# JuanTarrio/rebvo

Measured on AMD Instinct MI355X. Metric: frames/sec (DoG+extract+track+depth) 752x480 EuRoC, higher is better.
Workload: dtype f32 scale-space / f64 tracker+EKF

## Files before the change

rebvo_amd/csrc/stage_b.hip:

```cpp

#include <math.h>
#include <string.h>

#include <vector>

#include <type_traits>

#include "ctx.h"
#include "wave_reduce.h"

namespace edgehip {

struct RetuneArgs {
    SeqA *seqa;
    const int32_t *histo;
    float *retuned_out;
    int knum, nbins;
};
template <int NT>
__global__ __launch_bounds__(NT) void k_quantile(const KlSoA *kls, const int32_t *__restrict__ kns, SeqDev *seqs,
                                                 double smin, double smax, double pct, int nbins, const double *__restrict__ t_in, double fps,
                                                 RetuneArgs rt) {
    __shared__ int s_h[256];
    const int seq = blockIdx.x, tid = threadIdx.x;
// ... 502 lines not shown
    R[0] = 1.0 - B * (wy2 + wz2);
    R[4] = 1.0 - B * (wx2 + wz2);
    R[8] = 1.0 - B * (wx2 + wy2);
    double a = A * w[2], b = B * (w[0] * w[1]);
    R[1] = b - a; R[3] = b + a;
    a = A * w[1]; b = B * (w[0] * w[2]);
    R[2] = b + a; R[6] = b - a;
    a = A * w[0]; b = B * (w[1] * w[2]);
    R[5] = b - a; R[7] = b + a;
}
__device__ __noinline__ void so3_exp(const double w[3], double R[9]) {
    const double wv[3] = {w[0], w[1], w[2]};
    double Rr[9];
    so3_exp_inl(wv, Rr);
    for (int i = 0; i < 9; i++) R[i] = Rr[i];
}

__device__ __noinline__ void tvr_setup(SeqDev *sq, const double *X) {
    double R0[9], Rz[9];
    so3_exp(X + 3, R0);
    const double wz[3] = {0.0, 0.0, X[5]};
    so3_exp(wz, Rz);
    for (int i = 0; i < 9; i++) sq->Rt[i] = R0[i];
    sq->RM[0] = Rz[0]; sq->RM[1] = Rz[1]; sq->RM[2] = Rz[3]; sq->RM[3] = Rz[4];
    for (int i = 0; i < 3; i++) sq->Vt[i] = X[i];
}


__device__ __forceinline__ void tvr_setup2(SeqDev *sq, const double *X, const int lane, const bool zero = false, const int l0 = 0) {
    if (lane >= l0 && lane < l0 + 2) {
        const bool first = lane == l0;
        const double wv[3] = {first ? X[3] : 0.0, first ? X[4] : 0.0, X[5]};
        double R[9];
        so3_exp_inl(wv, R);
        double *Rt = zero ? sq->zRt : sq->Rt, *Vt = zero ? sq->zVt : sq->Vt, *RM = zero ? sq->zRM : sq->RM;
        if (first) {
            for (int i = 0; i < 9; i++) Rt[i] = R[i];
            for (int i = 0; i < 3; i++) Vt[i] = X[i];
        } else {
            RM[0] = R[0]; RM[1] = R[1]; RM[2] = R[3]; RM[3] = R[4];
        }
    }
}


struct TvrArgs {
    const KlSoA *kl_old;
    const KlSoA *kl_new;
    const int32_t *kn_old;
    const uint16_t *field16;
    const double *P0;
    double *resid;
    double *resid_carry;
    double *block_last;
    double *partials;
    double *block_last_z;
    double *partials_z;
    SeqDev *seq;
    const uint32_t *framecount;
    int w, h, cap, nblk, nseq;
    size_t f16stride;
    int f16tx;
    double zfm, max_r, match_thresh, k_huber, inv_k_huber;
    double inv_zfm;
    float ppx, ppy;
    uint32_t match_num_thresh;
    int write_mid;
    int use_grec;
    unsigned long long *fwd_key;
    const edgehip_kf_request *kf;
    double kf_match_mod, kf_match_cang, kf_rho_tol;
};

__device__ __forceinline__ double rsqrt_f64(double x) {
    double y = __builtin_amdgcn_rsq(x);
    const double hx = 0.5 * x;
    y = y * (1.5 - hx * y * y);
    y = y * (1.5 - hx * y * y);
    return x > 1e300 ? 0.0 : y;
}

__device__ __forceinline__ bool is_carry(double v) { return __double_as_longlong(v) == (long long)resid_carry_bits(); }

#ifndef EDGEHIP_TVR_MFMA
#define EDGEHIP_TVR_MFMA 0
#endif
#ifndef EDGEHIP_TVR_REF_ORDER
#define EDGEHIP_TVR_REF_ORDER 1
#endif
#ifndef EDGEHIP_TVR_ABL
#define EDGEHIP_TVR_ABL 0
#endif
template <bool REWEIGHT, bool PROCJF, bool GREC, bool KF = false>
__device__ __forceinline__ void tvr_body(const TvrArgs &a, const int seq, const int blk, const int tid) {
    constexpr int ABL = KF ? 0 : EDGEHIP_TVR_ABL;
    const int lane = tid & 63, wave = tid >> 6;
    SeqDev *sq = a.seq + seq;
    const int kn = a.kn_old[seq];
    if (blk * kTvrBlock >= kn) return;
    const KlSoA &ko = a.kl_old[seq];
    const int res_in = sq->res_cur, res_out = sq->lm_phase == 0 ? sq->res_t : sq->res_new;
    const double *rin = a.resid + ((size_t)res_in * a.nseq + seq) * a.cap;
    double *rout = a.resid + ((size_t)res_out * a.nseq + seq) * a.cap;
    const double carry_in_prev = a.resid_carry[((size_t)res_in * a.nseq + seq) * a.nblk + blk];
    const double marker = __longlong_as_double((long long)resid_carry_bits());

    constexpr int NW = kTvrThreads / 64;
    constexpr bool GRAM_MFMA = PROCJF && kTvrPasses == 1 && EDGEHIP_TVR_MFMA && !(ABL & 1);
    __shared__ double s_rows[GRAM_MFMA ? NW : 1][GRAM_MFMA ? 64 : 1][8];
    __shared__ double s_wlast[kTvrPasses][NW];
    __shared__ int s_whas[kTvrPasses][NW];
    double sums[kNumSums];
#pragma unroll
    for (int i = 0; i < kNumSums; i++) sums[i] = 0;

#pragma unroll 1
    for (int pass = 0; pass < kTvrPasses; pass++) {
        const int base = blk * kTvrBlock + pass * kTvrThreads;
        if (base >= kn) break;
        const int ikl = base + tid;
        double J[6] = {0, 0, 0, 0, 0, 0};
        double fm, dfx, dfy;
        double ptx, pty, ptz, pix, piy, rho_p, s_rho;
#if EDGEHIP_TVR_REF_ORDER
        double wgt_ref;
#else
        double inv_w2 = 1;
#endif
        int mid_f = -1;
        int status = 0;
        double fi = 0;
        double rho_own;
        if (ikl < kn) {
            s_rho = ldg(ko.s_rho, ikl);
            const int32_t mnum = ldg(ko.m_num, ikl);
            const float2 pm0 = ldg(ko.p_m, ikl);
            const double rho0 = ldg(ko.rho, ikl);
            rho_own = rho0;
            const float2 klm = ldg(ko.m_m, ikl);
            const float knm = ldg(ko.n_m, ikl);
            double rprev = 0;
            if (REWEIGHT && !(ABL & 16)) rprev = rin[ikl];
            const uint32_t fc = KF ? 0xFFFFFFFFu : a.framecount[seq];
            const uint32_t mthr = a.match_num_thresh < fc ? a.match_num_thresh : fc;
            const bool skip = s_rho > sq->s_rho_min_eval || (uint32_t)mnum < mthr;
            if (!skip) {
                const double sz = inv_mid(rho0);
                const double pz_zf0 = a.inv_zfm * sz;
                const double sx = pz_zf0 * (double)pm0.x, sy = pz_zf0 * (double)pm0.y;
                const double *R = sq->Rt, *V = sq->Vt;
                ptx = R[0] * sx; ptx += R[1] * sy; ptx += R[2] * sz; ptx = V[0] + ptx;
                pty = R[3] * sx; pty += R[4] * sy; pty += R[5] * sz; pty = V[1] + pty;
                ptz = R[6] * sx; ptz += R[7] * sy; ptz += R[8] * sz; ptz = V[2] + ptz;
                rho_p = inv_mid(ptz);
                const double pz_zf = a.zfm * rho_p;
                pix = pz_zf * ptx;
                piy = pz_zf * pty;
                const double px = pix + (double)a.ppx, py = piy + (double)a.ppy;
                const int x = cvt_trunc_sat_i32(px + 0.5), y = cvt_trunc_sat_i32(py + 0.5);
                dfx = 0; dfy = 0;
#if EDGEHIP_TVR_REF_ORDER
                wgt_ref = 1;
#endif
                if (REWEIGHT) {
                    if (is_carry(rprev)) rprev = carry_in_prev;
#if EDGEHIP_TVR_REF_ORDER
                    if (fabs(rprev) > a.k_huber) wgt_ref = div_mid(a.k_huber, fabs(rprev));
#else
                    if (fabs(rprev) > a.k_huber && !(ABL & 2)) { const double rk = fabs(rprev) * a.inv_k_huber; inv_w2 = rk * rk; }
#endif
                }
                fm = a.max_r;
                if (x < 1 || y < 1 || x >= a.w - 1 || y >= a.h - 1) {
                    status = 1;
                } else {
                    status = 3;
                    const float rmx = KF ? klm.x : (float)(sq->RM[0] * (double)klm.x + sq->RM[1] * (double)klm.y);
                    const float rmy = KF ? klm.y : (float)(sq->RM[2] * (double)klm.x + sq->RM[3] * (double)klm.y);
                    const uint32_t f = (ABL & 8) ? (uint32_t)(ikl + 1) : a.field16[(size_t)seq * a.f16stride + field16_index(x, y, a.f16tx)];
                    if (KF) {
                        if (f != 0u) {
                            const int ikf = (int)f - 1;
                            const KlSoA &kf = a.kl_new[seq];
                            const MatchRec fr = kf.rec[ikf];
                            const double f_rho = kf.rho[ikf], f_srho = kf.s_rho[ikf];
                            const double cang = (double)((klm.x * fr.m_mx + klm.y * fr.m_my) / knm);
                            const double rho_t = rho_p / a.kf[seq].Kr;
                            const bool reject = cang < a.kf_match_cang || (double)fabsf(knm / fr.n_m - 1) > a.kf_match_mod ||
                                                fabs(rho_t - f_rho) > a.kf_rho_tol * (f_srho + s_rho * rho_t / rho0);
                            if (!reject) {
                                const double dx = px - (double)fr.c_px, dy = py - (double)fr.c_py;
                                fi = dx * (double)fr.u_mx + dy * (double)fr.u_my;
// ... 39 lines not shown

        {
            const unsigned long long vmask = __ballot(status == 2);
            const unsigned long long below = vmask & ((1ull << lane) - 1ull);
            const int src = below ? 63 - __clzll(below) : 0;
            const double inh = __shfl(fi, src, 64);
            const int top = vmask ? 63 - __clzll(vmask) : 0;
            const double wl = __shfl(fi, top, 64);
            if (lane == 0) {
                s_whas[pass][wave] = vmask != 0;
                s_wlast[pass][wave] = wl;
            }
            __syncthreads();
            if (status == 3) {
                double v = marker;
                bool have = false;
                if (below) { v = inh; have = true; }
                for (int pp = pass; pp >= 0 && !have; pp--)
                    for (int pw = (pp == pass ? wave - 1 : NW - 1); pw >= 0 && !have; pw--)
                        if (s_whas[pp][pw]) { v = s_wlast[pp][pw]; have = true; }
                rout[ikl] = v;
            } else if (status == 2) {
                rout[ikl] = fi;
            } else if (status == 1) {
                rout[ikl] = a.max_r;
            } else if (ikl < kn) {
                rout[ikl] = 0.0;
            }
        }
        if (a.write_mid && ikl < kn) {
            stg(ko.m_id_f, ikl, mid_f);
            if (!KF && a.fwd_key && mid_f >= 0) atomicMax(&a.fwd_key[(size_t)seq * a.cap + mid_f], ord_bits(rho_own));
        }

        double fs = 0;
        if (status != 0) {
#if EDGEHIP_TVR_REF_ORDER
            if (REWEIGHT) { fm *= wgt_ref; dfx *= wgt_ref; dfy *= wgt_ref; }
#endif
            if (PROCJF) {
                double t0 = a.zfm * rho_p;
                J[0] = t0 * dfx;
                J[1] = t0 * dfy;
                t0 = rho_p * pix;
                J[2] = t0 * dfx;
                t0 = rho_p * piy;
                J[2] += t0 * dfy;
                J[3] = J[1] * ptz; J[3] += J[2] * pty;
                J[4] = J[0] * ptz; J[4] += J[2] * ptx;
                t0 = J[0] * pty;
                J[5] = -1 * t0; J[5] += J[1] * ptx;
            }
            const double qvel = (a.zfm * dfx * sq->Vt[0] + a.zfm * dfy * sq->Vt[1] + (pix * dfx + piy * dfy) * sq->Vt[2]);
#if EDGEHIP_TVR_REF_ORDER
            const double q_rho = REWEIGHT ? sqrt_ge1(s_rho * qvel * s_rho * qvel + 1) : s_rho;
            const double r_q = rcp_for_div_rn(q_rho);
            if (PROCJF) {
#pragma unroll
                for (int j = 0; j < 6; j++) J[j] = div_rn(J[j], q_rho, r_q);
            }
            fs = div_rn(fm, q_rho, r_q);
#else
            double inv_q;
            if (REWEIGHT) {
                const double sq = s_rho * qvel;
                inv_q = (ABL & 2) ? sq + inv_w2 : rsqrt_f64(sq * sq + inv_w2);
            } else {
                inv_q = 1.0 / s_rho;
            }
            if (PROCJF) {
#pragma unroll
                for (int j = 0; j < 6; j++) J[j] *= inv_q;
            }
            fs = fm * inv_q;
#endif
        } else if (!REWEIGHT && !KF && ikl < kn && s_rho == 0) {
            const double qnan = __longlong_as_double(0x7ff8000000000000ll);
            if (PROCJF) {
#pragma unroll
                for (int j = 0; j < 6; j++) J[j] = qnan;
            }
            fs = qnan;
        }
        if (GRAM_MFMA) {
            double2 *row = reinterpret_cast<double2 *>(&s_rows[wave][lane][0]);
            row[0] = make_double2(J[0], J[1]);
            row[1] = make_double2(J[2], J[3]);
            row[2] = make_double2(J[4], J[5]);
            row[3] = make_double2(fs, 0.0);
        } else {
            int ns = 0;
            if (PROCJF) {
#pragma unroll
                for (int i = 0; i < 6; i++)
#pragma unroll
                    for (int j = i; j < 6; j++) { const double pr = J[i] * J[j]; sums[ns] = kTvrPasses == 1 ? pr : sums[ns] + pr; ns++; }
#pragma unroll
                for (int i = 0; i < 6; i++) { const double pr = J[i] * fs; sums[ns] = kTvrPasses == 1 ? pr : sums[ns] + pr; ns++; }
            }
            { const double pr = fs * fs; const int at = PROCJF ? ns : kNumSums - 1; sums[at] = kTvrPasses == 1 ? pr : sums[at] + pr; }
        }
    }

    if (tid == 0) {
        double bl = marker;
        for (int pp = kTvrPasses - 1; pp >= 0 && is_carry(bl); pp--) {
            if (blk * kTvrBlock + pp * kTvrThreads >= kn) continue;
            for (int pw = NW - 1; pw >= 0; pw--)
                if (s_whas[pp][pw]) { bl = s_wlast[pp][pw]; break; }
        }
        a.block_last[(size_t)seq * a.nblk + blk] = bl;
    }

    __shared__ double s_red[NW][32];
    if (GRAM_MFMA) {
        typedef double v4d __attribute__((ext_vector_type(4)));
        __builtin_amdgcn_fence(__ATOMIC_RELEASE, "wavefront");
        __builtin_amdgcn_wave_barrier();
        const int m = (lane & 15) < 7 ? (lane & 15) : 7, kk = lane >> 4;
        const double *src = &s_rows[wave][kk][m];
        v4d acc = {0.0, 0.0, 0.0, 0.0};
#pragma unroll
        for (int st = 0; st < 16; st++) {
            const double v = src[st * 4 * 8];
            acc = __builtin_amdgcn_mfma_f64_16x16x4f64(v, v, acc, 0, 0, 0);
        }
        const int j = lane & 15;
#pragma unroll
        for (int r = 0; r < 2; r++) {
            const int i = (lane >> 4) + 4 * r;
            if (j < 7 && i <= j) {
                const int idx = j < 6 ? i * 6 - (i * (i - 1)) / 2 + (j - i) : (i < 6 ? 21 + i : 27);
                s_red[wave][idx] = acc[r];
            }
        }
    } else if (PROCJF && (ABL & 1)) {
        if (lane < kNumSums) s_red[wave][lane] = sums[lane % 4];
    } else if (PROCJF) {
        const int idx = wave_reduce28(sums, lane);
        if ((lane & 1) == 0) s_red[wave][idx] = sums[0];
    } else {
        double v = sums[kNumSums - 1];
#pragma unroll
        for (int o = 32; o > 0; o >>= 1) v += __shfl_xor(v, o, 64);
        if (lane == 0) s_red[wave][kNumSums - 1] = v;
    }
    __syncthreads();
    if (PROCJF ? tid < kNumSums : tid == kNumSums - 1) {
        double v = s_red[0][tid];
#pragma unroll
        for (int wv = 1; wv < NW; wv++) v += s_red[wv][tid];
        a.partials[((size_t)seq * a.nblk + blk) * kNumSums + tid] = v;
    }
}

template <bool REWEIGHT, bool PROCJF, bool GREC>
__global__ __launch_bounds__(kTvrThreads) void k_try_velrot(TvrArgs a) {
    tvr_body<REWEIGHT, PROCJF, GREC>(a, blockIdx.z, blockIdx.x, threadIdx.x);
}
__global__ __launch_bounds__(kTvrThreads) void k_try_velrot_kf(TvrArgs a) {
    tvr_body<true, true, false, true>(a, blockIdx.z, blockIdx.x, threadIdx.x);
}

template <bool REWEIGHT, bool PROCJF, bool GREC>
__device__ __forceinline__ void tvr_body_f32(const TvrArgs &a, const int seq, const int blk, const int tid) {
    static_assert(kTvrPasses == 1, "one KeyLine per thread");
    const int lane = tid & 63, wave = tid >> 6;
    SeqDev *sq = a.seq + seq;
    const int kn = a.kn_old[seq];
    if (blk * kTvrBlock >= kn) return;
    const KlSoA &ko = a.kl_old[seq];
    const int res_in = sq->res_cur, res_out = sq->lm_phase == 0 ? sq->res_t : sq->res_new;
    const double *rin = a.resid + ((size_t)res_in * a.nseq + seq) * a.cap;
    double *rout = a.resid + ((size_t)res_out * a.nseq + seq) * a.cap;
    const double carry_in_prev = a.resid_carry[((size_t)res_in * a.nseq + seq) * a.nblk + blk];
    const double marker = __longlong_as_double((long long)resid_carry_bits());
    constexpr int NW = kTvrThreads / 64;
    __shared__ float s_wlast[NW];
    __shared__ int s_whas[NW];
    float sums[kNumSums];
#pragma unroll
    for (int i = 0; i < kNumSums; i++) sums[i] = 0.f;

    const int ikl = blk * kTvrBlock + tid;
    float J[6] = {0, 0, 0, 0, 0, 0};
    float fm, dfx, dfy;
    float ptx, pty, ptz, pix, piy, rho_p;
    double s_rho;
    float wgt;
    int mid_f = -1, status = 0;
    float fi = 0;
    double rho_own;
    const float zf = (float)a.zfm, max_r = (float)a.max_r, k_huber = (float)a.k_huber, simil_t = (float)a.match_thresh;
    float Vt0, Vt1, Vt2;
    if (ikl < kn) {
        s_rho = ldg(ko.s_rho, ikl);
        const int32_t mnum = ldg(ko.m_num, ikl);
        const float2 pm0 = ldg(ko.p_m, ikl);
        const double rho0 = ldg(ko.rho, ikl);
        rho_own = rho0;
        const float2 klm = ldg(ko.m_m, ikl);
        const float knm = ldg(ko.n_m, ikl);
        double rprev_d = 0;
        if (REWEIGHT) rprev_d = rin[ikl];
        const uint32_t fc = a.framecount[seq];
        const uint32_t mthr = a.match_num_thresh < fc ? a.match_num_thresh : fc;
        const bool skip = s_rho > sq->s_rho_min_eval || (uint32_t)mnum < mthr;
        Vt0 = (float)sq->Vt[0]; Vt1 = (float)sq->Vt[1]; Vt2 = (float)sq->Vt[2];
        if (!skip) {
            const float sz = 1.f / (float)rho0;
            const float pz_zf0 = (1.f / zf) * sz;
            const float sx = pz_zf0 * pm0.x, sy = pz_zf0 * pm0.y;
            const double *Rd = sq->Rt;
            const float R0 = (float)Rd[0], R1 = (float)Rd[1], R2 = (float)Rd[2], R3 = (float)Rd[3], R4 = (float)Rd[4], R5 = (float)Rd[5],
                        R6 = (float)Rd[6], R7 = (float)Rd[7], R8 = (float)Rd[8];
            ptx = R0 * sx; ptx += R1 * sy; ptx += R2 * sz; ptx = Vt0 + ptx;
            pty = R3 * sx; pty += R4 * sy; pty += R5 * sz; pty = Vt1 + pty;
            ptz = R6 * sx; ptz += R7 * sy; ptz += R8 * sz; ptz = Vt2 + ptz;
            rho_p = 1.f / ptz;
            const float pz_zf = zf * rho_p;
            pix = pz_zf * ptx;
            piy = pz_zf * pty;
            const float px = pix + a.ppx, py = piy + a.ppy;
            const int x = cvt_trunc_sat_i32((double)px + 0.5), y = cvt_trunc_sat_i32((double)py + 0.5);
            dfx = 0; dfy = 0; wgt = 1;
            if (REWEIGHT) {
                if (is_carry(rprev_d)) rprev_d = carry_in_prev;
                const float rprev = (float)rprev_d;
                if (fabsf(rprev) > k_huber) wgt = k_huber / fabsf(rprev);
            }
            fm = max_r;
            if (x < 1 || y < 1 || x >= a.w - 1 || y >= a.h - 1) {
                status = 1;
            } else {
                status = 3;
                const float rmx = (float)sq->RM[0] * klm.x + (float)sq->RM[1] * klm.y;
                const float rmy = (float)sq->RM[2] * klm.x + (float)sq->RM[3] * klm.y;
                const uint32_t f = a.field16[(size_t)seq * a.f16stride + field16_index(x, y, a.f16tx)];
                {
                    const int ikf = f != 0u ? (int)f - 1 : 0;
                    float f_cpx, f_cpy, f_mx, f_my, f_ux, f_uy;
                    if (GREC) {
                        const float4 g = ldg(a.kl_new[seq].grec, ikf);
// ... 39 lines not shown
            bool have = false;
            if (below) { v = (double)inh; have = true; }
            for (int pw = wave - 1; pw >= 0 && !have; pw--)
                if (s_whas[pw]) { v = (double)s_wlast[pw]; have = true; }
            rout[ikl] = v;
        } else if (status == 2) {
            rout[ikl] = (double)fi;
        } else if (status == 1) {
            rout[ikl] = (double)max_r;
        } else if (ikl < kn) {
            rout[ikl] = 0.0;
        }
    }
    if (a.write_mid && ikl < kn) {
        stg(ko.m_id_f, ikl, mid_f);
        if (a.fwd_key && mid_f >= 0) atomicMax(&a.fwd_key[(size_t)seq * a.cap + mid_f], ord_bits(rho_own));
    }
    float fs = 0.f;
    if (status != 0) {
        if (REWEIGHT) { fm *= wgt; dfx *= wgt; dfy *= wgt; }
        if (PROCJF) {
            float t0 = zf * rho_p;
            J[0] = t0 * dfx;
            J[1] = t0 * dfy;
            t0 = rho_p * pix;
            J[2] = t0 * dfx;
            t0 = rho_p * piy;
            J[2] += t0 * dfy;
            J[3] = J[1] * ptz; J[3] += J[2] * pty;
            J[4] = J[0] * ptz; J[4] += J[2] * ptx;
            t0 = J[0] * pty;
            J[5] = -1.f * t0; J[5] += J[1] * ptx;
        }
        const double qvel = (double)(zf * dfx * Vt0 + zf * dfy * Vt1 + (pix * dfx + piy * dfy) * Vt2);
        const double q_rho = REWEIGHT ? sqrt_ge1(s_rho * qvel * s_rho * qvel + 1) : s_rho;
        const double r_q = rcp_for_div_rn(q_rho);
        if (PROCJF) {
#pragma unroll
            for (int j = 0; j < 6; j++) J[j] = (float)div_rn((double)J[j], q_rho, r_q);
        }
        fs = (float)div_rn((double)fm, q_rho, r_q);
    }
    {
        int ns = 0;
        if (PROCJF) {
#pragma unroll
            for (int i = 0; i < 6; i++)
#pragma unroll
                for (int j = i; j < 6; j++) sums[ns++] = J[i] * J[j];
#pragma unroll
            for (int i = 0; i < 6; i++) sums[ns++] = J[i] * fs;
        }
        sums[PROCJF ? ns : kNumSums - 1] = fs * fs;
    }
    if (tid == 0) {
        double bl = marker;
        for (int pw = NW - 1; pw >= 0; pw--)
            if (s_whas[pw]) { bl = (double)s_wlast[pw]; break; }
        a.block_last[(size_t)seq * a.nblk + blk] = bl;
    }
    __shared__ float s_red[NW][32];
    if (PROCJF) {
        const int idx = wave_reduce28_f32(sums, lane);
        if ((lane & 1) == 0) s_red[wave][idx] = sums[0];
    } else {
        float v = sums[kNumSums - 1];
#pragma unroll
        for (int o = 32; o > 0; o >>= 1) v += __shfl_xor(v, o, 64);
        if (lane == 0) s_red[wave][kNumSums - 1] = v;
    }
    __syncthreads();
    if (PROCJF ? tid < kNumSums : tid == kNumSums - 1) {
        float v = s_red[0][tid];
#pragma unroll
        for (int wv = 1; wv < NW; wv++) v += s_red[wv][tid];
        a.partials[((size_t)seq * a.nblk + blk) * kNumSums + tid] = (double)v;
    }
}
template <bool REWEIGHT, bool PROCJF, bool GREC>
__global__ __launch_bounds__(kTvrThreads) void k_try_velrot_f32(TvrArgs a) {
    tvr_body_f32<REWEIGHT, PROCJF, GREC>(a, blockIdx.z, blockIdx.x, threadIdx.x);
}

#ifndef EDGEHIP_TVR2_PARK
#define EDGEHIP_TVR2_PARK 1
#endif
template <bool PROCJF, bool GREC>
__device__ __forceinline__ void tvr2_body(const TvrArgs &a, const int seq, const int blk, const int tid) {
    const int lane = tid & 63, wave = tid >> 6;
    SeqDev *sq = a.seq + seq;
    const int kn = a.kn_old[seq];
    if (blk * kTvrBlock >= kn) return;
    static_assert(kTvrPasses == 1, "one KeyLine per thread");
    const KlSoA &ko = a.kl_old[seq];
    double *rout0 = a.resid + ((size_t)sq->res_t * a.nseq + seq) * a.cap;
    double *rout1 = a.resid + ((size_t)sq->res_new * a.nseq + seq) * a.cap;
    const double marker = __longlong_as_double((long long)resid_carry_bits());
    constexpr int NW = kTvrThreads / 64;
    __shared__ double s_wlast[2][NW];
    __shared__ int s_whas[2][NW];

    const int ikl = blk * kTvrBlock + tid;
    double fm[2], dfx[2], dfy[2], fi[2] = {0, 0};
    double ptx[2], pty[2], ptz[2], pix[2], piy[2], rho_p[2];
    int status[2] = {0, 0};
    double s_rho = 1;
    if (ikl < kn) {
        s_rho = ldg(ko.s_rho, ikl);
        const int32_t mnum = ldg(ko.m_num, ikl);
        const float2 pm0 = ldg(ko.p_m, ikl);
        const double rho0 = ldg(ko.rho, ikl);
        const float2 klm = ldg(ko.m_m, ikl);
        const float knm = ldg(ko.n_m, ikl);
        const uint32_t fc = a.framecount[seq];
        const uint32_t mthr = a.match_num_thresh < fc ? a.match_num_thresh : fc;
        const bool skip = s_rho > sq->s_rho_min_eval || (uint32_t)mnum < mthr;
        if (!skip) {
            const double sz = inv_mid(rho0);
            const double pz_zf0 = a.inv_zfm * sz;
            const double sx = pz_zf0 * (double)pm0.x, sy = pz_zf0 * (double)pm0.y;
            double px[2], py[2];
            bool inimg[2];
            size_t fidx[2];
            float rmx[2], rmy[2];
#pragma unroll
            for (int c = 0; c < 2; c++) {
                const double *R = c ? sq->Rt : sq->zRt, *V = c ? sq->Vt : sq->zVt, *RM = c ? sq->RM : sq->zRM;
                ptx[c] = R[0] * sx; ptx[c] += R[1] * sy; ptx[c] += R[2] * sz; ptx[c] = V[0] + ptx[c];
                pty[c] = R[3] * sx; pty[c] += R[4] * sy; pty[c] += R[5] * sz; pty[c] = V[1] + pty[c];
                ptz[c] = R[6] * sx; ptz[c] += R[7] * sy; ptz[c] += R[8] * sz; ptz[c] = V[2] + ptz[c];
                rho_p[c] = inv_mid(ptz[c]);
                const double pz_zf = a.zfm * rho_p[c];
                pix[c] = pz_zf * ptx[c];
                piy[c] = pz_zf * pty[c];
                px[c] = pix[c] + (double)a.ppx; py[c] = piy[c] + (double)a.ppy;
                const int x = x86_cvttsd2si(px[c] + 0.5), y = x86_cvttsd2si(py[c] + 0.5);
                inimg[c] = !(x < 1 || y < 1 || x >= a.w - 1 || y >= a.h - 1);
                fidx[c] = inimg[c] ? field16_index(x, y, a.f16tx) : (size_t)0;
                rmx[c] = (float)(RM[0] * (double)klm.x + RM[1] * (double)klm.y);
                rmy[c] = (float)(RM[2] * (double)klm.x + RM[3] * (double)klm.y);
                fm[c] = a.max_r;
                dfx[c] = 0; dfy[c] = 0;
                status[c] = inimg[c] ? 3 : 1;
            }
            const uint16_t *fld = a.field16 + (size_t)seq * a.f16stride;
            const uint32_t f0 = fld[fidx[0]], f1 = fld[fidx[1]];
            const bool hit0 = inimg[0] && f0 != 0u, hit1 = inimg[1] && f1 != 0u;
            const int ikf0 = hit0 ? (int)f0 - 1 : 0, ikf1 = hit1 ? (int)f1 - 1 : 0;
            float f_cpx[2], f_cpy[2], f_mx[2], f_my[2], f_ux[2] = {0, 0}, f_uy[2] = {0, 0};
            if (GREC) {
                const float4 g0 = ldg(a.kl_new[seq].grec, ikf0), g1 = ldg(a.kl_new[seq].grec, ikf1);
                f_cpx[0] = g0.x; f_cpy[0] = g0.y; f_mx[0] = g0.z; f_my[0] = g0.w;
                f_cpx[1] = g1.x; f_cpy[1] = g1.y; f_mx[1] = g1.z; f_my[1] = g1.w;
            } else {
                const MatchRec r0 = a.kl_new[seq].rec[ikf0], r1 = a.kl_new[seq].rec[ikf1];
                f_cpx[0] = r0.c_px; f_cpy[0] = r0.c_py; f_mx[0] = r0.m_mx; f_my[0] = r0.m_my; f_ux[0] = r0.u_mx; f_uy[0] = r0.u_my;
                f_cpx[1] = r1.c_px; f_cpy[1] = r1.c_py; f_mx[1] = r1.m_mx; f_my[1] = r1.m_my; f_ux[1] = r1.u_mx; f_uy[1] = r1.u_my;
            }
            const double p_n2 = (double)(knm * knm);
#pragma unroll
            for (int c = 0; c < 2; c++) {
                {
                    const double p_esc = (double)(rmx[c] * f_mx[c] + rmy[c] * f_my[c]);
                    if ((c ? hit1 : hit0) & !(fabs(p_esc - p_n2) > a.match_thresh * p_n2)) {
                        if (GREC) {
                            const float n2m = f_mx[c] * f_mx[c] + f_my[c] * f_my[c];
                            const float nm = sqrtf_mid(n2m);
                            div2_mid_f32(f_mx[c], f_my[c], nm, f_ux[c], f_uy[c]);
                        }
                        const double dx = px[c] - (double)f_cpx[c], dy = py[c] - (double)f_cpy[c];
                        fi[c] = dx * (double)f_ux[c] + dy * (double)f_uy[c];
                        dfx[c] = (double)f_ux[c];
                        dfy[c] = (double)f_uy[c];
                        fm[c] = fi[c];
                        status[c] = 2;
                    }
                }
            }
        }
    }

    unsigned long long below[2];
    double inh[2];
#pragma unroll
    for (int c = 0; c < 2; c++) {
        const unsigned long long vmask = __ballot(status[c] == 2);
        below[c] = vmask & ((1ull << lane) - 1ull);
        const int src = below[c] ? 63 - __clzll(below[c]) : 0;
        inh[c] = __shfl(fi[c], src, 64);
        const int top = vmask ? 63 - __clzll(vmask) : 0;
        const double wl = __shfl(fi[c], top, 64);
        if (lane == 0) {
            s_whas[c][wave] = vmask != 0;
            s_wlast[c][wave] = wl;
        }
    }
    __syncthreads();
#pragma unroll
    for (int c = 0; c < 2; c++) {
        double *rout = c ? rout1 : rout0;
        if (status[c] == 3) {
            double v = marker;
            bool have = false;
            if (below[c]) { v = inh[c]; have = true; }
            for (int pw = wave - 1; pw >= 0 && !have; pw--)
                if (s_whas[c][pw]) { v = s_wlast[c][pw]; have = true; }
            rout[ikl] = v;
        } else if (status[c] == 2) {
            rout[ikl] = fi[c];
        } else if (status[c] == 1) {
            rout[ikl] = a.max_r;
        } else if (ikl < kn) {
            rout[ikl] = 0.0;
        }
    }
    if (tid == 0) {
#pragma unroll
        for (int c = 0; c < 2; c++) {
            double bl = marker;
            for (int pw = NW - 1; pw >= 0; pw--)
                if (s_whas[c][pw]) { bl = s_wlast[c][pw]; break; }
            (c ? a.block_last : a.block_last_z)[(size_t)seq * a.nblk + blk] = bl;
        }
    }

    __shared__ double s_red[2][NW][32];
#if EDGEHIP_TVR2_PARK
    __shared__ double s_park[PROCJF ? 7 : 1][kTvrThreads];
#endif
    const double inv_q = rcp_for_div_rn(s_rho);
    double Jc[2][6], fmc[2];
#pragma unroll
    for (int c = 0; c < 2; c++) {
        double *J = Jc[c];
#pragma unroll
        for (int j = 0; j < 6; j++) J[j] = 0;
        fmc[c] = 0;
        if (status[c] != 0) {
            fmc[c] = fm[c];
            if (PROCJF) {
                double t0 = a.zfm * rho_p[c];
                J[0] = t0 * dfx[c];
                J[1] = t0 * dfy[c];
                t0 = rho_p[c] * pix[c];
                J[2] = t0 * dfx[c];
                t0 = rho_p[c] * piy[c];
                J[2] += t0 * dfy[c];
                J[3] = J[1] * ptz[c]; J[3] += J[2] * pty[c];
                J[4] = J[0] * ptz[c]; J[4] += J[2] * ptx[c];
                t0 = J[0] * pty[c];
                J[5] = -1 * t0; J[5] += J[1] * ptx[c];
#if EDGEHIP_TVR_REF_ORDER
#pragma unroll
                for (int j = 0; j < 6; j++) J[j] = div_rn(J[j], s_rho, inv_q);
#else
#pragma unroll
                for (int j = 0; j < 6; j++) J[j] *= inv_q;
#endif
            }
#if EDGEHIP_TVR_REF_ORDER
            fmc[c] = div_rn(fmc[c], s_rho, inv_q);
#else
            fmc[c] *= inv_q;
#endif
        } else if (ikl < kn && s_rho == 0) {
            const double qnan = __longlong_as_double(0x7ff8000000000000ll);
            if (PROCJF) {
#pragma unroll
                for (int j = 0; j < 6; j++) J[j] = qnan;
            }
            fmc[c] = qnan;
        }
    }
#if EDGEHIP_TVR2_PARK
    if (PROCJF) {
#pragma unroll
        for (int j = 0; j < 6; j++) s_park[j][tid] = Jc[1][j];
        s_park[6][tid] = fmc[1];
    }
#endif
#pragma unroll
    for (int c = 0; c < 2; c++) {
        if (PROCJF) {
            double J[6], f;
#if EDGEHIP_TVR2_PARK
            if (c == 1) {
#pragma unroll
                for (int j = 0; j < 6; j++) J[j] = s_park[j][tid];
                f = s_park[6][tid];
            } else
#endif
            {
#pragma unroll
                for (int j = 0; j < 6; j++) J[j] = Jc[c][j];
                f = fmc[c];
            }
            double sums[kNumSums];
            int ns = 0;
#pragma unroll
            for (int i = 0; i < 6; i++)
#pragma unroll
                for (int j = i; j < 6; j++) sums[ns++] = J[i] * J[j];
#pragma unroll
            for (int i = 0; i < 6; i++) sums[ns++] = J[i] * f;
            sums[ns] = f * f;
            const int idx = wave_reduce28(sums, lane);
            if ((lane & 1) == 0) s_red[c][wave][idx] = sums[0];
        } else {
            double v = fmc[c] * fmc[c];
#pragma unroll
            for (int o = 32; o > 0; o >>= 1) v += __shfl_xor(v, o, 64);
            if (lane == 0) s_red[c][wave][kNumSums - 1] = v;
        }
    }
    __syncthreads();
    if (wave < 2) {
        const int c = 1 - wave;
        if (PROCJF ? lane < kNumSums : lane == kNumSums - 1) {
            double v = s_red[c][0][lane];
#pragma unroll
            for (int wv = 1; wv < NW; wv++) v += s_red[c][wv][lane];
            (c ? a.partials : a.partials_z)[((size_t)seq * a.nblk + blk) * kNumSums + lane] = v;
        }
    }
}

template <bool PROCJF, bool GREC>
__device__ __forceinline__ void tvr2_body_f32(const TvrArgs &a, const int seq, const int blk, const int tid) {
    const int lane = tid & 63, wave = tid >> 6;
    SeqDev *sq = a.seq + seq;
    const int kn = a.kn_old[seq];
    if (blk * kTvrBlock >= kn) return;
    static_assert(kTvrPasses == 1, "one KeyLine per thread");
    const KlSoA &ko = a.kl_old[seq];
    double *rout0 = a.resid + ((size_t)sq->res_t * a.nseq + seq) * a.cap;
    double *rout1 = a.resid + ((size_t)sq->res_new * a.nseq + seq) * a.cap;
    const double marker = __longlong_as_double((long long)resid_carry_bits());
    constexpr int NW = kTvrThreads / 64;
    __shared__ float s_wlast[2][NW];
    __shared__ int s_whas[2][NW];
    const float zf = (float)a.zfm, max_r = (float)a.max_r, simil_t = (float)a.match_thresh;

    const int ikl = blk * kTvrBlock + tid;
    float fm[2] = {0, 0}, dfx[2] = {0, 0}, dfy[2] = {0, 0}, fi[2] = {0, 0};
    float ptx[2] = {0, 0}, pty[2] = {0, 0}, ptz[2] = {1, 1}, pix[2] = {0, 0}, piy[2] = {0, 0}, rho_p[2] = {1, 1};
    int status[2] = {0, 0};
    double s_rho = 1;
    if (ikl < kn) {
        s_rho = ldg(ko.s_rho, ikl);
        const int32_t mnum = ldg(ko.m_num, ikl);
        const float2 pm0 = ldg(ko.p_m, ikl);
        const double rho0 = ldg(ko.rho, ikl);
        const float2 klm = ldg(ko.m_m, ikl);
        const float knm = ldg(ko.n_m, ikl);
        const uint32_t fc = a.framecount[seq];
        const uint32_t mthr = a.match_num_thresh < fc ? a.match_num_thresh : fc;
        const bool skip = s_rho > sq->s_rho_min_eval || (uint32_t)mnum < mthr;
        if (!skip) {
            const float sz = 1.f / (float)rho0;
            const float pz_zf0 = (1.f / zf) * sz;
            const float sx = pz_zf0 * pm0.x, sy = pz_zf0 * pm0.y;
            float px[2], py[2];
            bool inimg[2];
            size_t fidx[2];
            float rmx[2], rmy[2];
#pragma unroll
            for (int c = 0; c < 2; c++) {
                const double *R = c ? sq->Rt : sq->zRt, *V = c ? sq->Vt : sq->zVt, *RM = c ? sq->RM : sq->zRM;
                ptx[c] = (float)R[0] * sx; ptx[c] += (float)R[1] * sy; ptx[c] += (float)R[2] * sz; ptx[c] = (float)V[0] + ptx[c];
                pty[c] = (float)R[3] * sx; pty[c] += (float)R[4] * sy; pty[c] += (float)R[5] * sz; pty[c] = (float)V[1] + pty[c];
                ptz[c] = (float)R[6] * sx; ptz[c] += (float)R[7] * sy; ptz[c] += (float)R[8] * sz; ptz[c] = (float)V[2] + ptz[c];
                rho_p[c] = 1.f / ptz[c];
                const float pz_zf = zf * rho_p[c];
                pix[c] = pz_zf * ptx[c];
                piy[c] = pz_zf * pty[c];
                px[c] = pix[c] + a.ppx; py[c] = piy[c] + a.ppy;
                const int x = x86_cvttsd2si((double)px[c] + 0.5), y = x86_cvttsd2si((double)py[c] + 0.5);
                inimg[c] = !(x < 1 || y < 1 || x >= a.w - 1 || y >= a.h - 1);
                fidx[c] = inimg[c] ? field16_index(x, y, a.f16tx) : (size_t)0;
                rmx[c] = (float)RM[0] * klm.x + (float)RM[1] * klm.y;
                rmy[c] = (float)RM[2] * klm.x + (float)RM[3] * klm.y;
                fm[c] = max_r;
                status[c] = inimg[c] ? 3 : 1;
            }
            const uint16_t *fld = a.field16 + (size_t)seq * a.f16stride;
            const uint32_t f0 = fld[fidx[0]], f1 = fld[fidx[1]];
            const bool hit0 = inimg[0] && f0 != 0u, hit1 = inimg[1] && f1 != 0u;
            const int ikf0 = hit0 ? (int)f0 - 1 : 0, ikf1 = hit1 ? (int)f1 - 1 : 0;
            float f_cpx[2], f_cpy[2], f_mx[2], f_my[2], f_ux[2] = {0, 0}, f_uy[2] = {0, 0};
            if (GREC) {
// ... 288 lines not shown
        }
    }
    if (tid == 0) {
#pragma unroll
        for (int c = 0; c < 2; c++) {
            if ((2 * blk + c) * kTvrBlock >= kn || 2 * blk + c >= a.nblk) continue;
            double bl = marker;
            for (int pw = NW - 1; pw >= 0; pw--)
                if (s_whas[c][pw]) { bl = s_wlast[c][pw]; break; }
            a.block_last[(size_t)seq * a.nblk + 2 * blk + c] = bl;
        }
    }
    double sums[kNumSums];
#pragma unroll
    for (int i = 0; i < kNumSums; i++) sums[i] = 0;
#pragma unroll
    for (int c = 0; c < 2; c++) {
        double J[6] = {0, 0, 0, 0, 0, 0};
        double fmc = fm[c];
        if (ikl[c] < kn) {
#if EDGEHIP_TVR_REF_ORDER
            fmc *= inv_w2[c]; dfx[c] *= inv_w2[c]; dfy[c] *= inv_w2[c];
#endif
            double t0 = a.zfm * rho_p[c];
            J[0] = t0 * dfx[c];
            J[1] = t0 * dfy[c];
            t0 = rho_p[c] * pix[c];
            J[2] = t0 * dfx[c];
            t0 = rho_p[c] * piy[c];
            J[2] += t0 * dfy[c];
            J[3] = J[1] * ptz[c]; J[3] += J[2] * pty[c];
            J[4] = J[0] * ptz[c]; J[4] += J[2] * ptx[c];
            t0 = J[0] * pty[c];
            J[5] = -1 * t0; J[5] += J[1] * ptx[c];
            const double qvel = (a.zfm * dfx[c] * V[0] + a.zfm * dfy[c] * V[1] + (pix[c] * dfx[c] + piy[c] * dfy[c]) * V[2]);
#if EDGEHIP_TVR_REF_ORDER
            const double q_rho = sqrt(s_rho[c] * qvel * s_rho[c] * qvel + 1), r_q = 1.0 / q_rho;
#pragma unroll
            for (int j = 0; j < 6; j++) J[j] = div_rn(J[j], q_rho, r_q);
            fmc = div_rn(fmc, q_rho, r_q);
#else
            const double sq_ = s_rho[c] * qvel;
            const double inv_q = rsqrt_f64(sq_ * sq_ + inv_w2[c]);
#pragma unroll
            for (int j = 0; j < 6; j++) J[j] *= inv_q;
            fmc *= inv_q;
#endif
        }
        int ns = 0;
#pragma unroll
        for (int i = 0; i < 6; i++)
#pragma unroll
            for (int j = i; j < 6; j++) sums[ns++] += J[i] * J[j];
#pragma unroll
        for (int i = 0; i < 6; i++) sums[ns++] += J[i] * fmc;
        sums[ns] += fmc * fmc;
    }
    __shared__ double s_red[NW][32];
    const int idx = wave_reduce28(sums, lane);
    if ((lane & 1) == 0) s_red[wave][idx] = sums[0];
    __syncthreads();
    if (tid < kNumSums) {
        double v = s_red[0][tid];
#pragma unroll
        for (int wv = 1; wv < NW; wv++) v += s_red[wv][tid];
        a.partials[((size_t)seq * a.nblk + 2 * blk) * kNumSums + tid] = v;
        if (2 * blk + 1 < a.nblk) a.partials[((size_t)seq * a.nblk + 2 * blk + 1) * kNumSums + tid] = 0.0;
    }
}

template <bool GREC>
__global__ __launch_bounds__(kTvrThreads) void k_try_velrot_rw2(TvrArgs a) {
    tvr_rw2_body<GREC>(a, blockIdx.z, blockIdx.x, threadIdx.x);
}
#endif

#ifndef EDGEHIP_TVR2_WAVES
#define EDGEHIP_TVR2_WAVES 0
#endif
template <bool PROCJF, bool GREC>
__global__ __launch_bounds__(kTvrThreads)
#if EDGEHIP_TVR2_WAVES > 0
__attribute__((amdgpu_waves_per_eu(EDGEHIP_TVR2_WAVES, EDGEHIP_TVR2_WAVES)))
#endif
void k_try_velrot2(TvrArgs a) {
    tvr2_body<PROCJF, GREC>(a, blockIdx.z, blockIdx.x, threadIdx.x);
}

__device__ __noinline__ void jacobi_eig6(const double Ain[36], double V[36], double e[6], double *A ) {
#pragma nounroll
    for (int i = 0; i < 36; i++) { A[i] = Ain[i]; V[i] = 0; }
#pragma nounroll
    for (int i = 0; i < 6; i++) V[i * 7] = 1;
    for (int sweep = 0; sweep < 30; sweep++) {
        double off = 0, diag = 0;
#pragma nounroll
        for (int p = 0; p < 6; p++) {
            diag += A[p * 7] * A[p * 7];
#pragma nounroll
            for (int q = p + 1; q < 6; q++) off += A[p * 6 + q] * A[p * 6 + q];
        }
        if (!(off > 1e-32 * diag) || !(off > 0)) break;
#pragma nounroll
        for (int p = 0; p < 5; p++)
#pragma nounroll
            for (int q = p + 1; q < 6; q++) {
                const double apq = A[p * 6 + q];
                if (apq == 0) continue;
                const double theta = (A[q * 7] - A[p * 7]) / (2 * apq);
                const double t = (theta >= 0 ? 1.0 : -1.0) / (fabs(theta) + sqrt(theta * theta + 1));
                const double c = 1 / sqrt(t * t + 1), s = t * c;
#pragma nounroll
                for (int k = 0; k < 6; k++) {
                    const double akp = A[k * 6 + p], akq = A[k * 6 + q];
                    A[k * 6 + p] = c * akp - s * akq;
                    A[k * 6 + q] = s * akp + c * akq;
                }
#pragma nounroll
                for (int k = 0; k < 6; k++) {
                    const double apk = A[p * 6 + k], aqk = A[q * 6 + k];
                    A[p * 6 + k] = c * apk - s * aqk;
                    A[q * 6 + k] = s * apk + c * aqk;
                }
#pragma nounroll
                for (int k = 0; k < 6; k++) {
                    const double vkp = V[k * 6 + p], vkq = V[k * 6 + q];
                    V[k * 6 + p] = c * vkp - s * vkq;
                    V[k * 6 + q] = s * vkp + c * vkq;
                }
            }
    }
#pragma nounroll
    for (int i = 0; i < 6; i++) e[i] = A[i * 7];
}

__device__ __noinline__ void svd_backsub6(const double A[36], const double b[6], double h[6], double *V, double *Awork,
                                          double *e, double *y) {
    jacobi_eig6(A, V, e, Awork);
    double smax = 0;
#pragma nounroll
    for (int i = 0; i < 6; i++) smax = fmax(smax, fabs(e[i]));
#pragma nounroll
    for (int i = 0; i < 6; i++) {
        double d = 0;
#pragma nounroll
        for (int k = 0; k < 6; k++) d += V[k * 6 + i] * b[k];
        const double inv = (fabs(e[i]) * 1e9 <= smax) ? 0.0 : 1.0 / e[i];
        y[i] = d * inv;
    }
#pragma nounroll
    for (int k = 0; k < 6; k++) {
        double d = 0;
#pragma nounroll
        for (int i = 0; i < 6; i++) d += V[k * 6 + i] * y[i];
        h[k] = d;
    }
}

__device__ __noinline__ void chol6(const double A[36], double L[36]) {
#pragma nounroll
    for (int i = 0; i < 36; i++) L[i] = A[i];
#pragma nounroll
    for (int col = 0; col < 6; col++) {
        double inv_diag = 1;
#pragma nounroll
        for (int row = col; row < 6; row++) {
// ... 1459 lines not shown
```

rebvo_amd/csrc/wave_reduce.h:

```cpp
#pragma once
#include "ctx.h"

namespace edgehip {

template <int N>
__device__ __forceinline__ void halve_step(double *v, int lane, int off) {
    const bool hi = (lane & off) != 0;
#pragma unroll
    for (int i = 0; i < N; i++) {
        const double send = hi ? v[i] : v[i + N];
        const double keep = hi ? v[i + N] : v[i];
        v[i] = keep + __shfl_xor(send, off, 64);
    }
}
template <int N, bool ROWS16>
__device__ __forceinline__ void halve_swap(double *v) {
#pragma unroll
    for (int i = 0; i < N; i++) {
        const unsigned alo = (unsigned)__double2loint(v[i]), ahi = (unsigned)__double2hiint(v[i]);
        const unsigned blo = (unsigned)__double2loint(v[i + N]), bhi = (unsigned)__double2hiint(v[i + N]);
        const auto rl = ROWS16 ? __builtin_amdgcn_permlane16_swap(alo, blo, false, false) : __builtin_amdgcn_permlane32_swap(alo, blo, false, false);
        const auto rh = ROWS16 ? __builtin_amdgcn_permlane16_swap(ahi, bhi, false, false) : __builtin_amdgcn_permlane32_swap(ahi, bhi, false, false);
        v[i] = __hiloint2double((int)rh[0], (int)rl[0]) + __hiloint2double((int)rh[1], (int)rl[1]);
    }
}
template <int CTRL>
__device__ __forceinline__ double dpp_mov_f64(double x) {
    const int lo = __builtin_amdgcn_update_dpp(0, __double2loint(x), CTRL, 0xf, 0xf, true);
    const int hi = __builtin_amdgcn_update_dpp(0, __double2hiint(x), CTRL, 0xf, 0xf, true);
    return __hiloint2double(hi, lo);
}
template <int N, int CTRL>
__device__ __forceinline__ void halve_dpp(double *v, int lane, int off) {
    const bool hi = (lane & off) != 0;
#pragma unroll
    for (int i = 0; i < N; i++) {
        const double send = hi ? v[i] : v[i + N];
        const double keep = hi ? v[i + N] : v[i];
        v[i] = keep + dpp_mov_f64<CTRL>(send);
    }
}
#ifndef EDGEHIP_REDUCE_DPP4
#define EDGEHIP_REDUCE_DPP4 1
#endif
__device__ __forceinline__ int dpp_xor4(int from_lower_rule, int from_upper_rule) {
    const int r = __builtin_amdgcn_update_dpp(0, from_lower_rule, 0x104, 0xf, 0xf, true);
    return __builtin_amdgcn_update_dpp(r, from_upper_rule, 0x114, 0xf, 0xa, false);
}
template <int N>
__device__ __forceinline__ void halve_dpp4(double *v, int lane) {
#if EDGEHIP_REDUCE_DPP4
    const bool hi = (lane & 4) != 0;
#pragma unroll
    for (int i = 0; i < N; i++) {
        const double keep = hi ? v[i + N] : v[i];
        const int lo = dpp_xor4(__double2loint(v[i]), __double2loint(v[i + N]));
        const int hw = dpp_xor4(__double2hiint(v[i]), __double2hiint(v[i + N]));
        v[i] = keep + __hiloint2double(hw, lo);
    }
#else
    halve_step<N>(v, lane, 4);
#endif
}
__device__ __forceinline__ int wave_reduce28(double (&s)[kNumSums], int lane) {
    double v[32];
#pragma unroll
    for (int i = 0; i < kNumSums; i++) v[i] = s[i];
    halve_swap<14, false>(v);
    halve_swap<7, true>(v);
    v[7] = 0.0;
    halve_dpp<4, 0x128>(v, lane, 8);
    halve_dpp4<2>(v, lane);
    halve_dpp<1, 0x4E>(v, lane, 2);
    v[0] += dpp_mov_f64<0xB1>(v[0]);
    s[0] = v[0];
    const int b1 = (lane >> 1) & 1, b2 = (lane >> 2) & 1, b3 = (lane >> 3) & 1, b4 = (lane >> 4) & 1, b5 = (lane >> 5) & 1;
    const int low = b1 + 2 * b2 + 4 * b3;
    return low == 7 ? 31 : low + 7 * b4 + 14 * b5;
}

template <int N, bool ROWS16>
__device__ __forceinline__ void halve_swap_f32(float *v) {
#pragma unroll
    for (int i = 0; i < N; i++) {
        const unsigned a = __float_as_uint(v[i]), b = __float_as_uint(v[i + N]);
        const auto r = ROWS16 ? __builtin_amdgcn_permlane16_swap(a, b, false, false) : __builtin_amdgcn_permlane32_swap(a, b, false, false);
        v[i] = __uint_as_float(r[0]) + __uint_as_float(r[1]);
    }
}
template <int CTRL>
__device__ __forceinline__ float dpp_mov_f32(float x) {
    return __int_as_float(__builtin_amdgcn_update_dpp(0, __float_as_int(x), CTRL, 0xf, 0xf, true));
}
template <int N, int CTRL>
__device__ __forceinline__ void halve_dpp_f32(float *v, int lane, int off) {
    const bool hi = (lane & off) != 0;
#pragma unroll
    for (int i = 0; i < N; i++) {
        const float send = hi ? v[i] : v[i + N];
        const float keep = hi ? v[i + N] : v[i];
        v[i] = keep + dpp_mov_f32<CTRL>(send);
    }
}
__device__ __forceinline__ int wave_reduce28_f32(float (&s)[kNumSums], int lane) {
    float v[32];
#pragma unroll
    for (int i = 0; i < kNumSums; i++) v[i] = s[i];
    halve_swap_f32<14, false>(v);
    halve_swap_f32<7, true>(v);
    v[7] = 0.f;
    halve_dpp_f32<4, 0x128>(v, lane, 8);
    {
        const bool hi = (lane & 4) != 0;
#pragma unroll
        for (int i = 0; i < 2; i++) {
            const float keep = hi ? v[i + 2] : v[i];
#if EDGEHIP_REDUCE_DPP4
            v[i] = keep + __int_as_float(dpp_xor4(__float_as_int(v[i]), __float_as_int(v[i + 2])));
#else
            const float send = hi ? v[i] : v[i + 2];
            v[i] = keep + __shfl_xor(send, 4, 64);
#endif
        }
    }
    halve_dpp_f32<1, 0x4E>(v, lane, 2);
    v[0] += dpp_mov_f32<0xB1>(v[0]);
    s[0] = v[0];
    const int b1 = (lane >> 1) & 1, b2 = (lane >> 2) & 1, b3 = (lane >> 3) & 1, b4 = (lane >> 4) & 1, b5 = (lane >> 5) & 1;
    const int low = b1 + 2 * b2 + 4 * b3;
    return low == 7 ? 31 : low + 7 * b4 + 14 * b5;
}

__device__ __forceinline__ int wave_reduce16(double (&v)[16], int lane) {
    halve_swap<8, false>(v);
    halve_swap<4, true>(v);
    halve_dpp<2, 0x128>(v, lane, 8);
    halve_dpp4<1>(v, lane);
    v[0] += dpp_mov_f64<0x4E>(v[0]);
    v[0] += dpp_mov_f64<0xB1>(v[0]);
    return 8 * ((lane >> 5) & 1) + 4 * ((lane >> 4) & 1) + 2 * ((lane >> 3) & 1) + ((lane >> 2) & 1);
}

}
```

Baseline: 131,300.

## Compute tracker Gram reductions with f64 4x4x4 MFMA via LDS row staging

Replaces the per-lane 28-product accumulation plus cross-lane butterfly reduction in the velocity/rotation tracker kernels with a shared wave_gram7 helper. The helper stages each lane's 7-element Jacobian/residual row in LDS and accumulates the 7x7 Gram matrix using f64 4x4x4 MFMA instructions with four independent accumulators. It is enabled by default in both tvr and tvr2 paths, and the tvr2 register-parking path is removed. Occupancy hints (waves_per_eu 8 and 7) are added to the kernels, trading register budget for more resident waves, with LDS traffic and extra shared memory as the cost.

```diff
diff --git a/rebvo_amd/csrc/stage_b.hip b/rebvo_amd/csrc/stage_b.hip
--- a/rebvo_amd/csrc/stage_b.hip
+++ b/rebvo_amd/csrc/stage_b.hip
@@ -608,9 +608,6 @@
 
 __device__ __forceinline__ bool is_carry(double v) { return __double_as_longlong(v) == (long long)resid_carry_bits(); }
 
-#ifndef EDGEHIP_TVR_MFMA
-#define EDGEHIP_TVR_MFMA 0
-#endif
 #ifndef EDGEHIP_TVR_REF_ORDER
 #define EDGEHIP_TVR_REF_ORDER 1
 #endif
@@ -632,8 +629,10 @@
     const double marker = __longlong_as_double((long long)resid_carry_bits());
 
     constexpr int NW = kTvrThreads / 64;
-    constexpr bool GRAM_MFMA = PROCJF && kTvrPasses == 1 && EDGEHIP_TVR_MFMA && !(ABL & 1);
-    __shared__ double s_rows[GRAM_MFMA ? NW : 1][GRAM_MFMA ? 64 : 1][8];
+    constexpr bool GRAM = PROCJF && !(ABL & 1);
+    static_assert(!GRAM || kTvrPasses == 1, "wave_gram7 sums one row per lane");
+    __shared__ double s_rows[GRAM ? NW * kGramDoubles : 1];
+    double row[7] = {0, 0, 0, 0, 0, 0, 0};
     __shared__ double s_wlast[kTvrPasses][NW];
     __shared__ int s_whas[kTvrPasses][NW];
     double sums[kNumSums];
@@ -839,12 +838,10 @@
             }
             fs = qnan;
         }
-        if (GRAM_MFMA) {
-            double2 *row = reinterpret_cast<double2 *>(&s_rows[wave][lane][0]);
-            row[0] = make_double2(J[0], J[1]);
-            row[1] = make_double2(J[2], J[3]);
-            row[2] = make_double2(J[4], J[5]);
-            row[3] = make_double2(fs, 0.0);
+        if (GRAM) {
+#pragma unroll
+            for (int j = 0; j < 6; j++) row[j] = J[j];
+            row[6] = fs;
         } else {
             int ns = 0;
             if (PROCJF) {
@@ -870,32 +867,10 @@
     }
 
     __shared__ double s_red[NW][32];
-    if (GRAM_MFMA) {
-        typedef double v4d __attribute__((ext_vector_type(4)));
-        __builtin_amdgcn_fence(__ATOMIC_RELEASE, "wavefront");
-        __builtin_amdgcn_wave_barrier();
-        const int m = (lane & 15) < 7 ? (lane & 15) : 7, kk = lane >> 4;
-        const double *src = &s_rows[wave][kk][m];
-        v4d acc = {0.0, 0.0, 0.0, 0.0};
-#pragma unroll
-        for (int st = 0; st < 16; st++) {
-            const double v = src[st * 4 * 8];
-            acc = __builtin_amdgcn_mfma_f64_16x16x4f64(v, v, acc, 0, 0, 0);
-        }
-        const int j = lane & 15;
-#pragma unroll
-        for (int r = 0; r < 2; r++) {
-            const int i = (lane >> 4) + 4 * r;
-            if (j < 7 && i <= j) {
-                const int idx = j < 6 ? i * 6 - (i * (i - 1)) / 2 + (j - i) : (i < 6 ? 21 + i : 27);
-                s_red[wave][idx] = acc[r];
-            }
-        }
-    } else if (PROCJF && (ABL & 1)) {
+    if (GRAM) {
+        wave_gram7(row, s_rows + wave * kGramDoubles, s_red[wave], lane);
+    } else if (PROCJF) {
         if (lane < kNumSums) s_red[wave][lane] = sums[lane % 4];
-    } else if (PROCJF) {
-        const int idx = wave_reduce28(sums, lane);
-        if ((lane & 1) == 0) s_red[wave][idx] = sums[0];
     } else {
         double v = sums[kNumSums - 1];
 #pragma unroll
@@ -912,10 +887,10 @@
 }
 
 template <bool REWEIGHT, bool PROCJF, bool GREC>
-__global__ __launch_bounds__(kTvrThreads) void k_try_velrot(TvrArgs a) {
+__global__ __launch_bounds__(kTvrThreads) __attribute__((amdgpu_waves_per_eu(8))) void k_try_velrot(TvrArgs a) {
     tvr_body<REWEIGHT, PROCJF, GREC>(a, blockIdx.z, blockIdx.x, threadIdx.x);
 }
-__global__ __launch_bounds__(kTvrThreads) void k_try_velrot_kf(TvrArgs a) {
+__global__ __launch_bounds__(kTvrThreads) __attribute__((amdgpu_waves_per_eu(8))) void k_try_velrot_kf(TvrArgs a) {
     tvr_body<true, true, false, true>(a, blockIdx.z, blockIdx.x, threadIdx.x);
 }
 
@@ -1121,9 +1096,6 @@
     tvr_body_f32<REWEIGHT, PROCJF, GREC>(a, blockIdx.z, blockIdx.x, threadIdx.x);
 }
 
-#ifndef EDGEHIP_TVR2_PARK
-#define EDGEHIP_TVR2_PARK 1
-#endif
 template <bool PROCJF, bool GREC>
 __device__ __forceinline__ void tvr2_body(const TvrArgs &a, const int seq, const int blk, const int tid) {
     const int lane = tid & 63, wave = tid >> 6;
@@ -1264,9 +1236,7 @@
     }
 
     __shared__ double s_red[2][NW][32];
-#if EDGEHIP_TVR2_PARK
-    __shared__ double s_park[PROCJF ? 7 : 1][kTvrThreads];
-#endif
+    __shared__ double s_rows[PROCJF ? NW * kGramDoubles : 1];
     const double inv_q = rcp_for_div_rn(s_rho);
     double Jc[2][6], fmc[2];
 #pragma unroll
@@ -1311,40 +1281,11 @@
             fmc[c] = qnan;
         }
     }
-#if EDGEHIP_TVR2_PARK
-    if (PROCJF) {
-#pragma unroll
-        for (int j = 0; j < 6; j++) s_park[j][tid] = Jc[1][j];
-        s_park[6][tid] = fmc[1];
-    }
-#endif
 #pragma unroll
     for (int c = 0; c < 2; c++) {
         if (PROCJF) {
-            double J[6], f;
-#if EDGEHIP_TVR2_PARK
-            if (c == 1) {
-#pragma unroll
-                for (int j = 0; j < 6; j++) J[j] = s_park[j][tid];
-                f = s_park[6][tid];
-            } else
-#endif
-            {
-#pragma unroll
-                for (int j = 0; j < 6; j++) J[j] = Jc[c][j];
-                f = fmc[c];
-            }
-            double sums[kNumSums];
-            int ns = 0;
-#pragma unroll
-            for (int i = 0; i < 6; i++)
-#pragma unroll
-                for (int j = i; j < 6; j++) sums[ns++] = J[i] * J[j];
-#pragma unroll
-            for (int i = 0; i < 6; i++) sums[ns++] = J[i] * f;
-            sums[ns] = f * f;
-            const int idx = wave_reduce28(sums, lane);
-            if ((lane & 1) == 0) s_red[c][wave][idx] = sums[0];
+            const double row[7] = {Jc[c][0], Jc[c][1], Jc[c][2], Jc[c][3], Jc[c][4], Jc[c][5], fmc[c]};
+            wave_gram7(row, s_rows + wave * kGramDoubles, s_red[c][wave], lane);
         } else {
             double v = fmc[c] * fmc[c];
 #pragma unroll
@@ -1799,6 +1740,8 @@
 __global__ __launch_bounds__(kTvrThreads)
 #if EDGEHIP_TVR2_WAVES > 0
 __attribute__((amdgpu_waves_per_eu(EDGEHIP_TVR2_WAVES, EDGEHIP_TVR2_WAVES)))
+#else
+__attribute__((amdgpu_waves_per_eu(7)))
 #endif
 void k_try_velrot2(TvrArgs a) {
     tvr2_body<PROCJF, GREC>(a, blockIdx.z, blockIdx.x, threadIdx.x);
diff --git a/rebvo_amd/csrc/wave_reduce.h b/rebvo_amd/csrc/wave_reduce.h
--- a/rebvo_amd/csrc/wave_reduce.h
+++ b/rebvo_amd/csrc/wave_reduce.h
@@ -79,6 +79,26 @@
     return low == 7 ? 31 : low + 7 * b4 + 14 * b5;
 }
 
+constexpr int kGramStride = 7;
+constexpr int kGramDoubles = 64 * kGramStride;
+__device__ __forceinline__ void wave_gram7(const double (&row)[7], double *rows, double *red, int lane) {
+#pragma unroll
+    for (int e = 0; e < 7; e++) rows[lane * kGramStride + e] = row[e];
+    __builtin_amdgcn_fence(__ATOMIC_RELEASE, "wavefront");
+    __builtin_amdgcn_wave_barrier();
+    const int x = lane & 3, p = (lane >> 3) & 1, q = (lane >> 2) & 1, y = lane >> 4;
+    const int ea = 4 * p + x < 7 ? 4 * p + x : 6, eb = 4 * q + x < 7 ? 4 * q + x : 6;
+    const double *pa = rows + y * kGramStride + ea, *pb = rows + y * kGramStride + eb;
+    double acc[4] = {0.0, 0.0, 0.0, 0.0};
+#pragma unroll
+    for (int s = 0; s < 16; s++)
+        acc[s & 3] = __builtin_amdgcn_mfma_f64_4x4x4f64(pa[s * 4 * kGramStride], pb[s * 4 * kGramStride], acc[s & 3], 0, 0, 0);
+    const double d = (acc[0] + acc[1]) + (acc[2] + acc[3]);
+    const int i = 4 * p + y, j = 4 * q + x;
+    if (i <= j && j < 7) red[j < 6 ? i * 6 - (i * (i - 1)) / 2 + (j - i) : (i < 6 ? 21 + i : 27)] = d;
+    __builtin_amdgcn_wave_barrier();
+}
+
 template <int N, bool ROWS16>
 __device__ __forceinline__ void halve_swap_f32(float *v) {
 #pragma unroll
```

New measurement: 133,600 (median of 4 runs). About the same (+1.7%).
